# fhausmann/deepgrp

Measured on AMD Instinct MI355X. Metric: Mbp/sec predicted (whole node) at window=200 stride=50, 5-class, higher is better.
Workload: dtype f16

## Files before the change

deepgrp_amd/__main__.py:

```python
#!/usr/bin/env python3
from __future__ import annotations

import argparse
import logging
import os
import sys
from typing import Iterator, List, TextIO, Tuple

import numpy as np

logging.basicConfig()
_LOG = logging.getLogger(__name__)


def _read_multi_fasta(filestream: TextIO) -> Iterator[Tuple[str, str]]:
    from .fasta import read_multi_fasta_lines
    _LOG.debug("Reading FASTA file.")
    yield from read_multi_fasta_lines(filestream)


def _predict(dnasequence: str, model, options, step_size: int, use_mss: bool) -> Tuple[np.ndarray, int]:
    from .pipeline import ContigPipeline, upload_sequence
    _LOG.debug("One hot encoding sequence.")
    start_pos, d_idx = upload_sequence(dnasequence.encode("utf-8"))
# ... 379 lines not shown

    @staticmethod
    def _pipeline(args, options, model):
        from .pipeline import ContigPipeline
        pipe = ContigPipeline(model, args.step_size, options.batch_size, options.min_mss_len, options.xdrop_len,
                              use_mss=not args.no_use_mss, precise=getattr(args, "precise", False),
                              fast=getattr(args, "fast", False))
        _LOG.info("Forward kernel: %s", "plain fp32 kernels (more units than the fused kernels take)" if getattr(model, "fp32_only", False)
                  else "fused, split operands (fp32-grade)" if pipe.split else "fused, fp16 operands")
        return pipe

    _last_count = 0

    @staticmethod
    def _counted(records, _cb):
        from .fasta import DeviceRecord
        CommandLineParser._last_count = 0
        for header, rec in records:
            CommandLineParser._last_count += max(rec.length, 0) + max(rec.startpos, 0) if isinstance(rec, DeviceRecord) else len(rec)
            yield header, rec

    @staticmethod
    def _predict_tracked(pipe, runner, filename, records, outstream, kept, files, spec) -> int:
        from .evaluation import record_name
        from .runner import rows_text, rows_text_batch
        from .tracks import record_texts
        try:
            if _LOG.isEnabledFor(logging.DEBUG):
                bases = 0
                for chrom, (header, rec) in enumerate(records):
                    name = record_name(filename, header)
                    sink = lambda merged, startpos: files.write(record_texts(pipe, merged, startpos, name, spec, chrom))
                    rows, n = CommandLineParser._predict_staged(pipe, header, rec, sink)
                    if n == 0 and spec.bigwig:
# ... 406 lines not shown
```

deepgrp_amd/_lib.py:

```python
from __future__ import annotations

import ctypes as C
import os

_HERE = os.path.dirname(os.path.abspath(__file__))
LIB_PATH = os.path.join(_HERE, "libdeepgrp_hip.so")

i64, i32, vp, cint = C.c_int64, C.c_int32, C.c_void_p, C.c_int


class DgrpError(RuntimeError):
    """A libdeepgrp_hip call failed (message from dgrp_last_error())."""


class Segment(C.Structure):
    _fields_ = [("start", C.c_int64), ("end", C.c_int64), ("label", C.c_int32), ("contig", C.c_int32)]


_SIGNATURES = {
    "dgrp_abi_version": (cint, []),
    "dgrp_last_error": (C.c_char_p, []),
    "dgrp_device_info": (cint, [C.c_char_p, C.c_size_t, C.POINTER(cint), C.POINTER(i64)]),
    "dgrp_strip_n": (cint, [vp, i64, C.POINTER(i64), C.POINTER(i64)]),
    "dgrp_encode": (cint, [vp, i64, vp, vp]),
# ... 43 lines not shown
    "dgrp_forward_merge_record_workspace_bytes": (i64, [vp, i64, i64]),
    "dgrp_forward_reference_workspace_bytes": (i64, [vp, i64]),
    "dgrp_forward_windows_reference": (cint, [vp, vp, i64, i64, i64, i64, vp, vp, i64, vp]),
    "dgrp_get_max": (cint, [vp, i64, vp, i64, i64, i64, i64, vp]),
    "dgrp_scores": (cint, [vp, i64, cint, vp, vp, vp]),
    "dgrp_softmax_labels": (cint, [vp, i64, cint, vp, vp, vp, i64, vp]),
    "dgrp_mss_workspace_bytes": (i64, [i64]),
    "dgrp_mss_labels": (cint, [vp, vp, i64, cint, cint, cint, vp, vp, vp, i64, vp]),
    "dgrp_mss_segments_host": (cint, [vp, i64, vp, i64, C.POINTER(i64)]),
    "dgrp_mss_batch_workspace_bytes": (i64, [i64, i64]),
    "dgrp_mss_labels_batch": (cint, [vp, vp, i64, i64, vp, cint, cint, cint, vp, vp, i64, vp]),
    "dgrp_segments_workspace_bytes": (i64, [i64]),
    "dgrp_segments": (cint, [vp, i64, i64, i32, vp, i64, vp, vp, i64, vp]),
    "dgrp_record_workspace_bytes": (i64, [vp, i64, i64, cint]),
    "dgrp_predict_record": (cint, [vp, vp, i64, i64, i64, cint, cint, cint, i64, i32, vp, i64, C.POINTER(i64), vp, i64, vp]),
    "dgrp_batch_workspace_bytes": (i64, [vp, i64, vp, i64]),
    "dgrp_predict_batch": (cint, [vp, vp, i64, vp, vp, vp, vp, i64, i64, cint, cint, vp, i64, C.POINTER(i64), vp, i64, vp]),
    "dgrp_batch_rows": (i64, [i64, vp]),
    "dgrp_predict_batch_probs": (cint, [vp, vp, i64, vp, vp, vp, vp, i64, i64, cint, cint, vp, i64, C.POINTER(i64), vp, i64, vp, vp]),
    "dgrp_confusion_matrix": (cint, [vp, vp, i64, cint, vp, vp, vp]),
    "dgrp_filter_segments": (cint, [vp, vp, i64, i64, vp]),
    "dgrp_eval_workspace_bytes": (i64, [i64, i64]),
    "dgrp_paint_rows_batch": (cint, [vp, i64, vp, vp, vp, vp, vp, vp, i64, vp]),
    "dgrp_row_hits_batch": (cint, [vp, i64, vp, vp, vp, vp, vp, vp, vp, i64, vp]),
    "dgrp_row_scores_workspace_bytes": (i64, [i64, i64]),
    "dgrp_row_scores_batch": (cint, [vp, cint, i64, vp, vp, vp, vp, vp, vp, vp, i64, vp]),
    "dgrp_format_bed_bound": (i64, [i64, i64]),
    "dgrp_format_bed_rows": (cint, [vp, vp, i64, cint, vp, vp, i64, cint, vp, i64, C.POINTER(i64)]),
    "dgrp_inflate_raw_host": (cint, [vp, i64, vp, i64, C.POINTER(i64), C.POINTER(i64), C.POINTER(cint)]),
    "dgrp_inflate_workspace_bytes": (i64, [i64]),
# ... 43 lines not shown
```

deepgrp_amd/csrc/api.hip:

```cpp
#include "dgrp_model.h"

#include <stdarg.h>
#include <string.h>

#include <algorithm>
#include <vector>
#include <mutex>

static thread_local char g_err[512] = "";

void dgrp_set_error(const char *fmt, ...)
{
    va_list ap;
    va_start(ap, fmt);
    vsnprintf(g_err, sizeof(g_err), fmt, ap);
    va_end(ap);
}

DGRP_EXPORT int dgrp_abi_version(void) { return DGRP_ABI_VERSION; }
DGRP_EXPORT const char *dgrp_last_error(void) { return g_err; }

DGRP_EXPORT int dgrp_device_info(char *name, size_t name_cap, int *cu_count, int64_t *hbm_bytes)
{
    int dev = 0;
// ... 802 lines not shown
    l.count = take(8);
    l.fwd_bytes = record_forward_bytes(m, nwin);
    l.fwd = take(l.fwd_bytes);
    l.post_bytes = std::max<int64_t>(std::max<int64_t>(use_mss ? dgrp_mss_workspace_bytes(n) : 4096, dgrp_segments_workspace_bytes(n)), 4096);
    l.post = take(l.post_bytes);
    l.bytes = p;
    return l;
}

DGRP_EXPORT int64_t dgrp_record_workspace_bytes(const dgrp_model *m, int64_t n, int64_t s, int use_mss)
{
    if (!m || n < 0 || s < 1) return 0;
    return record_carve(m, n, s, use_mss).bytes;
}

DGRP_EXPORT int dgrp_predict_record(const dgrp_model *m, const uint8_t *d_idx, int64_t n, int64_t s, int64_t batch,
                                    int min_mss_len, int xdrop_len, int use_mss, int64_t offset, int32_t contig,
                                    dgrp_segment *d_records, int64_t cap, int64_t *h_count, void *d_work,
                                    int64_t work_bytes, void *stream_)
{
    hipStream_t stream = (hipStream_t)stream_;
    DGRP_REQUIRE(m && n >= 0 && s >= 1 && batch >= 1 && cap >= 0 && h_count, "dgrp_predict_record: bad arguments");
    *h_count = 0;
    if (n == 0) return DGRP_OK;
    DGRP_REQUIRE(d_idx && d_work && (cap == 0 || d_records), "dgrp_predict_record: NULL pointer");
    const record_layout l = record_carve(m, n, s, use_mss);
    if (work_bytes < l.bytes) {
        dgrp_set_error("dgrp_predict_record: workspace %lld < %lld bytes", (long long)work_bytes, (long long)l.bytes);
        return DGRP_ENOMEM;
    }
    char *w = (char *)d_work;
    float *out = (float *)(w + l.out);
    int8_t *labels = (int8_t *)(w + l.labels);
    int64_t *d_count = (int64_t *)(w + l.count);
    DGRP_HIP(hipMemsetAsync(out, 0, (size_t)n * m->C * 4, stream));
    int rc = dgrp_forward_merge_record(m, d_idx, n, s, batch, out, w + l.fwd, l.fwd_bytes, stream);
    if (rc) return rc;
    if (use_mss) {
        rc = dgrp_scores(out, n, m->C, (double *)(w + l.scores), (int8_t *)(w + l.cls), stream);
        if (rc) return rc;
        rc = dgrp_mss_labels((const double *)(w + l.scores), (const int8_t *)(w + l.cls), n, m->C, min_mss_len, xdrop_len,
                             labels, nullptr, w + l.post, l.post_bytes, stream);
    } else {
        rc = dgrp_softmax_labels(out, n, m->C, nullptr, labels, w + l.post, l.post_bytes, stream);
    }
    if (rc) return rc;
    rc = dgrp_segments(labels, n, offset, contig, d_records, cap, d_count, w + l.post, l.post_bytes, stream);
    if (rc) return rc;
    DGRP_HIP(hipMemcpyAsync(h_count, d_count, 8, hipMemcpyDeviceToHost, stream));
    DGRP_HIP(hipStreamSynchronize(stream));
    return DGRP_OK;
}

int dgrp_batch_marks(const int64_t *d_start, const int64_t *d_len, int64_t nrec, int64_t total_n, uint8_t *d_marks,
                     double *d_scores, int8_t *d_cls, hipStream_t stream);
int dgrp_batch_segments(const int8_t *d_labels, const uint8_t *d_marks, int64_t total_n, const int64_t *d_start, int64_t nrec,
                        const int64_t *d_startpos, const int32_t *d_contig, dgrp_segment *d_records, int64_t cap,
                        int64_t *d_count, void *d_work, int64_t work_bytes, hipStream_t stream);

struct batch_layout {
    int64_t out, scores, cls, labels, marks, count, recs, wgf, start, len, spos, contig, post, post_bytes, avg, pl, bytes;
};

static batch_layout batch_carve(const dgrp_model *m, int64_t nrec, int64_t total_rows, int64_t total_windows)
{
    batch_layout l;
// ... 142 lines not shown
```

deepgrp_amd/csrc/fasta_kernels.hip:

```cpp
#include "dgrp_common.h"
#include "scan.h"
#include <vector>
#include <algorithm>
#include <string.h>

__device__ __forceinline__ uint32_t fasta_class_of(uint32_t c)
{
    uint32_t l = c | 0x20u;
    return l == 'a' ? 0u : l == 'c' ? 1u : l == 'g' ? 2u : l == 't' ? 3u : 4u;
}

__global__ void __launch_bounds__(256) fasta_count_kernel(const uint8_t *__restrict__ raw, int64_t n, uint64_t *__restrict__ tilecnt,
                                                          unsigned long long *__restrict__ g)
{
    __shared__ uint64_t lds[4];
    const int64_t base = (int64_t)blockIdx.x * SCAN_TILE;
    uint64_t c = 0;
    bool bad = false;
    for (int j = 0; j < 8; ++j) {
        const int64_t i = base + j * 256 + threadIdx.x;
        if (i < n) {
            const uint32_t b = raw[i];
            const bool lineend = b == '\n' || b == '\r';
            c += lineend ? 0 : 1;
// ... 233 lines not shown
    if (word > 0) DGRP_HIP(hipMemcpyAsync(htiles.data(), tiles_base, (size_t)word * 8, hipMemcpyDeviceToHost, stream));
    DGRP_HIP(hipStreamSynchronize(stream));
    for (int64_t r = 0; r < nrec; ++r) {
        int64_t *info = h_info + 4 * r;
        if (h_len[r] == 0) { info[0] = 1; info[1] = 0; info[2] = 0; info[3] = 0; continue; }
        const unsigned long long *g = hg.data() + (size_t)r * 32;
        const int64_t tot = small[(size_t)r] ? (int64_t)g[3] : (int64_t)htiles[(size_t)grand_at[(size_t)r]];
        info[0] = g[0] ? 0 : 1;
        info[1] = tot;
        if (g[2] == 0) { info[2] = tot; info[3] = -tot; }
        else { info[2] = (int64_t)g[1]; info[3] = (int64_t)g[2] - (int64_t)g[1]; }
    }
    return DGRP_OK;
}

__global__ void __launch_bounds__(256) fasta_gt_kernel(const uint8_t *__restrict__ raw, int64_t n, int64_t cap,
                                                       unsigned long long *__restrict__ count, int64_t *__restrict__ list)
{
    const int64_t nvec = n / 16;
    for (int64_t v = (int64_t)blockIdx.x * blockDim.x + threadIdx.x; v <= nvec; v += (int64_t)gridDim.x * blockDim.x) {
        const int64_t p0 = v * 16;
        union { uint4 q; uint8_t b[16]; } u;
        uint8_t *b = u.b;
        int m = 16;
        if (v < nvec) {
            u.q = *(const uint4 *)(raw + p0);
        } else {
            m = (int)(n - p0);
            for (int j = 0; j < m; ++j) b[j] = raw[p0 + j];
        }
// ... 185 lines not shown
```

deepgrp_amd/fasta.py:

```python
from __future__ import annotations

import io
import mmap
import threading
import os
from typing import Iterator, List, Optional, TextIO, Tuple, Union

_DELETE = b"\n\r"
_ODD_WHITESPACE = (b" ", b"\t", b"\x0b", b"\x0c", b"\x1c", b"\x1d", b"\x1e", b"\x1f", b"\x85")


class LineLoop:

    __slots__ = ("header", "sequence", "opened", "key", "last_key")

    def __init__(self):
        self.header = ""
        self.sequence: List[str] = []
        self.opened = 0
        self.key = self.last_key = None

    def feed(self, lines, tag=None) -> Iterator[Tuple[str, str]]:
        for line in lines:
            line = line.strip()
# ... 100 lines not shown
    UPLOAD_STATS["bytes"] += int(size)
    UPLOAD_STATS["uploads"] += 1
    if size <= _SLAB:
        import numpy as np
        return torch.from_numpy(np.fromfile(path, dtype=np.uint8, count=size, offset=offset)).to(dev)
    key = (dev.index if dev.index is not None else torch.cuda.current_device())
    if key not in _UPLOAD:
        from concurrent.futures import ThreadPoolExecutor
        _UPLOAD[key] = ([torch.empty(_SLAB, dtype=torch.uint8, pin_memory=True) for _ in range(_NSLAB)], torch.cuda.Stream(device=dev),
                        ThreadPoolExecutor(max_workers=_NSLAB, thread_name_prefix="dgrp-upload"))
    slabs, copy, pool = _UPLOAD[key]
    with _UPLOAD_LOCK:
        return _upload_through(path, size, dev, slabs, copy, pool, offset)


def _upload_through(path, size: int, dev, slabs, copy, pool, offset: int = 0):
    import torch
    nslab = len(slabs)
    views = [b.numpy() for b in slabs]
    d_file = torch.empty(size, dtype=torch.uint8, device=dev)
    copy.wait_stream(torch.cuda.current_stream())
    fd = os.open(path, os.O_RDONLY)

    def reader(j):
        sent = None
        with torch.cuda.stream(copy):
            for o in range(j * _SLAB, size, nslab * _SLAB):
                want = min(_SLAB, size - o)
                if sent is not None:
                    sent.synchronize()
                got = 0
                while got < want:
                    k = os.preadv(fd, [views[j][got:want]], offset + o + got)
                    if not k:
                        raise OSError(f"{path}: shorter than its size at open ({offset + o + got} of {offset + size} bytes)")
                    got += k
                d_file[o:o + want].copy_(slabs[j][:want], non_blocking=True)
                sent = torch.cuda.Event()
                sent.record(copy)
        if sent is not None:
            sent.synchronize()

    try:
        jobs = [pool.submit(reader, j) for j in range(nslab)]
        err = None
        for job in jobs:
            try:
                job.result()
            except BaseException as e:
                err = err or e
        if err is not None:
            raise err
    finally:
        os.close(fd)
    torch.cuda.current_stream().wait_stream(copy)
    return d_file


def _device_chunks(L, d_file, size: int):
    import ctypes as C

    import numpy as np
    import torch

    from ._lib import check
    from .pipeline import stream_ptr
    cap = 4096
    while True:
        wb = L.dgrp_fasta_chunks_workspace_bytes(cap)
        work = torch.empty(wb, dtype=torch.uint8, device=d_file.device)
        st, lf, n = np.empty(cap, np.int64), np.empty(cap, np.int64), C.c_int64()
# ... 180 lines not shown
            work = torch.empty(wb, dtype=torch.uint8, device=dev)
            check(L.dgrp_fasta_encode_batch(d_raw.data_ptr(), c1 - c0, off.ctypes.data, ln.ctypes.data, d_idx.data_ptr(),
                                            infos.ctypes.data, work.data_ptr(), wb, stream_ptr()), "dgrp_fasta_encode_batch")
            del work
        if not keep_raw:
            d_raw = None
        grp = ChunkGroup()
        grp.c0, grp.c1, grp.starts, grp.head_ends, grp.body0s, grp.cand = c0, c1, starts, head_ends, body0s, cand
        grp.info, grp.d_idx, grp.d_raw = infos.tolist(), d_idx, d_raw
        del d_idx, d_raw
        yield grp
        del grp
        c0 = c1


def _ingest_range(L, dev, path, mm, r0: int, r1: int, group_bytes: int, group_records: int, d_file=None):
    loop = LineLoop()
    for grp in _chunk_groups(L, dev, path, mm, r0, r1, group_bytes, group_records, d_file=d_file):
        starts, head_ends, g0 = grp.starts, grp.head_ends, grp.starts[grp.c0]
        for i, c in enumerate(range(grp.c0, grp.c1)):
            a, b = r0 + starts[c], r0 + starts[c + 1]
            if grp.plain(i):
                for header, seq in loop.flush():
                    yield loop.last_key, header, seq
                header = mm[a:r0 + head_ends[c]].decode("ascii").strip()[1:]
                if header:
                    st, kept = grp.info[i][2], grp.info[i][3]
                    lo = grp.body0s[i] - g0 + st
                    yield (a, 0), header, DeviceRecord(st, None, kept, grp.d_idx, lo)
                continue
            for header, seq in loop.feed(_text_lines(mm[a:b]), tag=a):
# ... 5 lines not shown
```

deepgrp_amd/pipeline.py:

```python
from __future__ import annotations

import ctypes as C
from typing import NamedTuple, Optional, Tuple

import numpy as np
import torch

from ._lib import check, lib
from .fasta import DeviceRecord

SEGMENT_DTYPE = np.dtype([("start", "<i8"), ("end", "<i8"), ("label", "<i4"), ("contig", "<i4")])
ROW_SCORE_DTYPE = np.dtype([("sum", "<u8"), ("bases", "<i8"), ("agree", "<i8"), ("qmin", "<u4"), ("pad", "<u4")])


def require_gpu() -> torch.device:
    if not torch.cuda.is_available():
        raise RuntimeError("deepgrp_amd needs an AMD MI355X (gfx950) visible to PyTorch-ROCm; "
                           "there is no CPU fallback")
    return torch.device("cuda", torch.cuda.current_device())


def stream_ptr() -> int:
    return torch.cuda.current_stream().cuda_stream

# ... 373 lines not shown
        wb = L.dgrp_record_workspace_bytes(self.handle, n, self.step, int(self.use_mss))
        work = torch.empty(wb, dtype=torch.uint8, device=dev)
        cap = max(1024, n // 64)
        count = C.c_int64(0)
        while True:
            rec = torch.empty(cap * SEGMENT_DTYPE.itemsize, dtype=torch.uint8, device=dev)
            check(L.dgrp_predict_record(self.handle, _ptr(d_idx), n, self.step, self.batch, self.min_mss_len,
                                        self.xdrop_len, int(self.use_mss), int(startpos), int(contig), _ptr(rec), cap,
                                        C.byref(count), _ptr(work), wb, stream_ptr()), "dgrp_predict_record")
            if count.value <= cap:
                break
            cap = int(count.value)
        host = rec[: count.value * SEGMENT_DTYPE.itemsize].cpu().numpy()
        return host.view(SEGMENT_DTYPE).copy()

    def batchable(self) -> bool:
        return self.use_mss and self.event_log is None and not self.fp32 and not getattr(self.model, "fp32_only", False)

    def run_batch(self, d_base: torch.Tensor, offsets, lengths, startposes, contigs, d_probs: Optional[torch.Tensor] = None) -> np.ndarray:
        L = lib()
        nrec = len(lengths)
        if nrec == 0:
            return np.zeros(0, SEGMENT_DTYPE)
        off = np.ascontiguousarray(offsets, np.int64)
        ln = np.ascontiguousarray(lengths, np.int64)
        sp = np.ascontiguousarray(startposes, np.int64)
        cg = np.ascontiguousarray(contigs, np.int32)
        dev = d_base.device
        wb = L.dgrp_batch_workspace_bytes(self.handle, nrec, ln.ctypes.data, self.step)
        if wb <= 0:
# ... 259 lines not shown
```

deepgrp_amd/runner.py:

```python
from __future__ import annotations

import collections
import os
import threading
from concurrent.futures import ThreadPoolExecutor
from typing import Iterable, Iterator, List, NamedTuple, Tuple

import numpy as np
import torch

from .fasta import DeviceRecord
from .pipeline import ContigPipeline, record_indices

class _Tracked(NamedTuple):
    name: str
    rec: object
    chrom: int = 0


class _TrackedBatch(list):
    chrom0 = 0


class _Scored(NamedTuple):
    name: str
    rec: object
# ... 51 lines not shown
        return ""
    return _format(["{}\t{}\t".format(filename, h).encode("utf-8", "surrogateescape") for h in headers], True, rows)


class RecordRunner:

    def __init__(self, pipe: ContigPipeline, workers: int = 0, max_bases: int = 1 << 29, tracks=None):
        self.pipe = pipe
        self.tracks = tracks
        self.workers = workers or int(os.environ.get("DGRP_CLI_WORKERS", "16"))
        self.max_bases = max_bases
        m = pipe.model
        self._T, self._UP = m.vecsize, (m.units + 31) // 32 * 32

    def run_record(self, rec, contig: int = 0) -> np.ndarray:
        if isinstance(rec, DeviceRecord):
            startpos, d_idx = record_indices(rec)
            return self.pipe.run_idx(d_idx, startpos, contig)
        return self.pipe.run(rec, contig)

    def run_tracked(self, rec, name: str, chrom: int = 0):
        from .pipeline import SEGMENT_DTYPE
        from .tracks import empty_texts, record_texts
        startpos, d_idx = record_indices(rec)
        if d_idx.numel() == 0:
            return np.zeros(0, SEGMENT_DTYPE), empty_texts(self.tracks, name, startpos)
        merged = self.pipe.merged(d_idx)
        texts = record_texts(self.pipe, merged, startpos, name, self.tracks, chrom)
        return self.pipe.segments(self.pipe.labels(merged), startpos), texts

# ... 11 lines not shown

    def _batch_cost(self, n: int) -> int:
        cost = 80 * n
        m = self.pipe.model
        if self.tracks is not None:
            cost += 4 * m.classes * (n + 64) + len(self.tracks.classes) * (n // self.tracks.bin + 2) * (4 + 12 + 32)
        if m.attention:
            cost += len(range(0, n - self._T, self.pipe.step)) * self._T * (self._UP * 4 + m.classes * 4)
        return cost

    def work_items(self, records: Iterable[Tuple[object, object]]) -> Iterator[Tuple[object, object]]:
        group: List[Tuple[object, DeviceRecord]] = []
        cost = 0
        batchable = self.pipe.batchable()
        for key, rec in records:
            small = batchable and isinstance(rec, DeviceRecord) and rec.base is not None and 1 <= rec.length <= SMALL_RECORD
            if small:
                c = self._batch_cost(rec.length)
                if group and (group[0][1].base is not rec.base or len(group) >= BATCH_RECORDS or cost + c > BATCH_BYTES):
                    yield _BATCH, group
                    group, cost = [], 0
                group.append((key, rec))
                cost += c
            else:
                if group:
                    yield _BATCH, group
                    group, cost = [], 0
                yield key, rec
        if group:
            yield _BATCH, group
# ... 19 lines not shown
                texts = self.pipe.batch_track_texts(d_probs, row0, np.ascontiguousarray(lengths, np.int64), startposes,
                                                    [k[1] for k, _r in item], self.tracks, item.chrom0 if self.tracks.bigwig else 0)
            return [k for k, _r in item], rows, scores, texts
        if isinstance(item, list):
            rows = self.pipe.run_batch(item[0][1].base, [r.offset for _k, r in item], [r.length for _k, r in item],
                                       [r.startpos for _k, r in item], list(range(len(item))))
            return [k for k, _r in item], rows
        return self.run_record(item)

    @staticmethod
    def _size(item) -> int:
        if isinstance(item, (_Tracked, _Scored)):
            item = item.rec
        if isinstance(item, list):
            return sum(r.length for _k, r in item)
        return item.d_idx.numel() if isinstance(item, DeviceRecord) else len(item)

    def in_order(self, items: Iterable[Tuple[object, object]]) -> Iterator[Tuple[object, object]]:
        dev = torch.cuda.current_device() if torch.cuda.is_available() else None
        local = threading.local()
        taken = iter(range(self.workers))

        def task(item):
            if dev is None:
                return self.run_item(item)
            if not hasattr(local, "stream"):
                torch.cuda.set_device(dev)
                local.stream = _worker_stream(dev, next(taken))
            with torch.cuda.stream(local.stream):
                out = self.run_item(item)
# ... 67 lines not shown
```

include/deepgrp_hip.h:

```cpp
#ifndef DEEPGRP_HIP_H_
#define DEEPGRP_HIP_H_

#include <stddef.h>
#include <stdint.h>

#ifdef __cplusplus
extern "C" {
#endif

#define DGRP_OK 0
#define DGRP_EINVAL (-1)
#define DGRP_EHIP (-2)
#define DGRP_ENOMEM (-3)
#define DGRP_ENODEV (-4)

#define DGRP_ABI_VERSION 1

typedef struct dgrp_segment {
    int64_t start;
    int64_t end;
    int32_t label;
    int32_t contig;
} dgrp_segment;

// ... 147 lines not shown
                          dgrp_track_totals *h_totals, void *d_work, int64_t work_bytes, void *stream);

int64_t dgrp_zlib_bound(int64_t nblk, int64_t in_bytes);
int64_t dgrp_zlib_workspace_bytes(int64_t nblk, int level);
int dgrp_zlib_compress_batch(const uint8_t *d_in, int64_t in_bytes, const void *d_rows, int64_t stride, int64_t nblk, int level,
                             uint8_t *d_out, int64_t out_cap, int64_t *d_sizes, int64_t *h_out_bytes, void *d_work, int64_t work_bytes,
                             void *stream);
int dgrp_zlib_compress_host(const uint8_t *h_in, int64_t in_bytes, const void *h_rows, int64_t stride, int64_t nblk, int level,
                            uint8_t *h_out, int64_t out_cap, int64_t *h_sizes, int64_t *h_out_bytes);

int64_t dgrp_record_workspace_bytes(const dgrp_model *m, int64_t n, int64_t s, int use_mss);
int dgrp_predict_record(const dgrp_model *m, const uint8_t *d_idx, int64_t n, int64_t s, int64_t batch,
                        int min_mss_len, int xdrop_len, int use_mss, int64_t offset, int32_t contig,
                        dgrp_segment *d_records, int64_t cap, int64_t *h_count, void *d_work, int64_t work_bytes,
                        void *stream);

int64_t dgrp_batch_workspace_bytes(const dgrp_model *m, int64_t nrec, const int64_t *h_n, int64_t s);
int dgrp_predict_batch(const dgrp_model *m, const uint8_t *d_idx, int64_t nrec, const int64_t *h_idx_off,
                       const int64_t *h_n, const int64_t *h_startpos, const int32_t *h_contig, int64_t s, int64_t batch,
                       int min_mss_len, int xdrop_len, dgrp_segment *d_records, int64_t cap, int64_t *h_count,
                       void *d_work, int64_t work_bytes, void *stream);

int64_t dgrp_batch_rows(int64_t nrec, const int64_t *h_n);
int dgrp_predict_batch_probs(const dgrp_model *m, const uint8_t *d_idx, int64_t nrec, const int64_t *h_idx_off,
                             const int64_t *h_n, const int64_t *h_startpos, const int32_t *h_contig, int64_t s, int64_t batch,
                             int min_mss_len, int xdrop_len, dgrp_segment *d_records, int64_t cap, int64_t *h_count,
                             void *d_work, int64_t work_bytes, void *stream, float *d_probs);

int dgrp_confusion_matrix(const int8_t *d_true, const int8_t *d_pred, int64_t n, int ncls, int64_t *d_cnf,
                          int *d_bad, void *stream);
// ... 61 lines not shown
```

Baseline: 560.2.

## Stream large FASTA records in slabs and overlap encoding and GRU with upload

Large single-record FASTA files are now uploaded in slabs, and each slab is encoded on the device as soon as it arrives. GRU forward launches start on the windows already available while the rest of the file is still uploading, with a fallback that recomputes everything if the leading-N guess was wrong. This is meant to hide file upload and encoding time behind model compute for big chromosomes. It adds a new host/device handshake (ready flags, events, spin waits) and more complex record accounting, and it risks redundant work when the start-position guess misses.

```diff
diff --git a/deepgrp_amd/__main__.py b/deepgrp_amd/__main__.py
--- a/deepgrp_amd/__main__.py
+++ b/deepgrp_amd/__main__.py
@@ -417,10 +417,16 @@
 
     @staticmethod
     def _counted(records, _cb):
-        from .fasta import DeviceRecord
+        from .fasta import DeviceRecord, StreamedRecord
         CommandLineParser._last_count = 0
+
+        def add(n):
+            CommandLineParser._last_count += n
         for header, rec in records:
-            CommandLineParser._last_count += max(rec.length, 0) + max(rec.startpos, 0) if isinstance(rec, DeviceRecord) else len(rec)
+            if isinstance(rec, StreamedRecord) and rec.info is None:
+                rec.on_settle = lambda r: add(max(r.info[3], 0) + max(r.info[2], 0))
+            else:
+                add(max(rec.length, 0) + max(rec.startpos, 0) if isinstance(rec, DeviceRecord) else len(rec))
             yield header, rec
 
     @staticmethod
diff --git a/deepgrp_amd/_lib.py b/deepgrp_amd/_lib.py
--- a/deepgrp_amd/_lib.py
+++ b/deepgrp_amd/_lib.py
@@ -81,6 +81,11 @@
     "dgrp_segments": (cint, [vp, i64, i64, i32, vp, i64, vp, vp, i64, vp]),
     "dgrp_record_workspace_bytes": (i64, [vp, i64, i64, cint]),
     "dgrp_predict_record": (cint, [vp, vp, i64, i64, i64, cint, cint, cint, i64, i32, vp, i64, C.POINTER(i64), vp, i64, vp]),
+    "dgrp_stream_record_min_bytes": (i64, []),
+    "dgrp_stream_record_workspace_bytes": (i64, [vp, i64, i64, cint]),
+    "dgrp_predict_record_streamed": (cint, [vp, vp, i64, i64, vp, vp, vp, i64, i64, vp, i64, i64, cint, cint, cint, i32, vp, i64,
+                                            C.POINTER(i64), vp, vp, i64, vp]),
+    "dgrp_fasta_encode_slabs": (cint, [vp, i64, i64, vp, vp, vp, vp, i64, vp]),
     "dgrp_batch_workspace_bytes": (i64, [vp, i64, vp, i64]),
     "dgrp_predict_batch": (cint, [vp, vp, i64, vp, vp, vp, vp, i64, i64, cint, cint, vp, i64, C.POINTER(i64), vp, i64, vp]),
     "dgrp_batch_rows": (i64, [i64, vp]),
diff --git a/deepgrp_amd/csrc/api.hip b/deepgrp_amd/csrc/api.hip
--- a/deepgrp_amd/csrc/api.hip
+++ b/deepgrp_amd/csrc/api.hip
@@ -1,6 +1,7 @@
 #include "dgrp_model.h"
 
 #include <stdarg.h>
+#include <sched.h>
 #include <string.h>
 
 #include <algorithm>
@@ -840,6 +841,29 @@
     return record_carve(m, n, s, use_mss).bytes;
 }
 
+static int record_post(const dgrp_model *m, const record_layout &l, char *w, int64_t n, int min_mss_len, int xdrop_len, int use_mss,
+                       int64_t offset, int32_t contig, dgrp_segment *d_records, int64_t cap, int64_t *h_count, hipStream_t stream)
+{
+    float *out = (float *)(w + l.out);
+    int8_t *labels = (int8_t *)(w + l.labels);
+    int64_t *d_count = (int64_t *)(w + l.count);
+    int rc;
+    if (use_mss) {
+        rc = dgrp_scores(out, n, m->C, (double *)(w + l.scores), (int8_t *)(w + l.cls), stream);
+        if (rc) return rc;
+        rc = dgrp_mss_labels((const double *)(w + l.scores), (const int8_t *)(w + l.cls), n, m->C, min_mss_len, xdrop_len,
+                             labels, nullptr, w + l.post, l.post_bytes, stream);
+    } else {
+        rc = dgrp_softmax_labels(out, n, m->C, nullptr, labels, w + l.post, l.post_bytes, stream);
+    }
+    if (rc) return rc;
+    rc = dgrp_segments(labels, n, offset, contig, d_records, cap, d_count, w + l.post, l.post_bytes, stream);
+    if (rc) return rc;
+    DGRP_HIP(hipMemcpyAsync(h_count, d_count, 8, hipMemcpyDeviceToHost, stream));
+    DGRP_HIP(hipStreamSynchronize(stream));
+    return DGRP_OK;
+}
+
 DGRP_EXPORT int dgrp_predict_record(const dgrp_model *m, const uint8_t *d_idx, int64_t n, int64_t s, int64_t batch,
                                     int min_mss_len, int xdrop_len, int use_mss, int64_t offset, int32_t contig,
                                     dgrp_segment *d_records, int64_t cap, int64_t *h_count, void *d_work,
@@ -857,25 +881,140 @@
     }
     char *w = (char *)d_work;
     float *out = (float *)(w + l.out);
-    int8_t *labels = (int8_t *)(w + l.labels);
-    int64_t *d_count = (int64_t *)(w + l.count);
     DGRP_HIP(hipMemsetAsync(out, 0, (size_t)n * m->C * 4, stream));
     int rc = dgrp_forward_merge_record(m, d_idx, n, s, batch, out, w + l.fwd, l.fwd_bytes, stream);
     if (rc) return rc;
-    if (use_mss) {
-        rc = dgrp_scores(out, n, m->C, (double *)(w + l.scores), (int8_t *)(w + l.cls), stream);
+    return record_post(m, l, w, n, min_mss_len, xdrop_len, use_mss, offset, contig, d_records, cap, h_count, stream);
+}
+
+int dgrp_fasta_slab_begin(unsigned long long *d_st, int64_t n, hipStream_t stream);
+int dgrp_fasta_slab_ingest(const uint8_t *d_raw, int64_t a, int64_t b, int64_t n, uint8_t *d_idx, unsigned long long *d_st,
+                           uint64_t *d_tiles, hipStream_t stream);
+void dgrp_fasta_slab_info(const unsigned long long *h_st, int64_t *h_info);
+
+DGRP_EXPORT int64_t dgrp_stream_record_min_bytes(void)
+{
+    static const int64_t v = [] {
+        const char *e = getenv("DGRP_STREAM_MIN_BYTES");
+        if (!e || !e[0]) return (int64_t)(32ll << 20);
+        if (e[0] == 'o' || e[0] == 'O' || e[0] == '-') return (int64_t)-1;
+        return (int64_t)atoll(e);
+    }();
+    return v;
+}
+
+static int64_t round_windows()
+{
+    int dev = 0, cus = 0;
+    if (hipGetDevice(&dev) != hipSuccess || hipDeviceGetAttribute(&cus, hipDeviceAttributeMultiprocessorCount, dev) != hipSuccess || cus < 1)
+        cus = 256;
+    return 32ll * cus;
+}
+
+static int64_t stream_record_fasta_bytes(int64_t body_bytes)
+{
+    return dgrp_align_up(dgrp_fasta_workspace_bytes(body_bytes), 256);
+}
+
+DGRP_EXPORT int64_t dgrp_stream_record_workspace_bytes(const dgrp_model *m, int64_t body_bytes, int64_t s, int use_mss)
+{
+    if (!m || body_bytes < 0 || s < 1) return 0;
+    return record_carve(m, body_bytes, s, use_mss).bytes + stream_record_fasta_bytes(body_bytes);
+}
+
+DGRP_EXPORT int dgrp_predict_record_streamed(const dgrp_model *m, const uint8_t *d_body, int64_t body_bytes, int64_t nslab,
+                                             const int64_t *h_slab_end, void *const *h_events, const int32_t *h_ready,
+                                             int64_t startpos, int64_t range_windows, uint8_t *d_idx, int64_t s, int64_t batch,
+                                             int min_mss_len, int xdrop_len, int use_mss, int32_t contig, dgrp_segment *d_records,
+                                             int64_t cap, int64_t *h_count, int64_t *h_info, void *d_work, int64_t work_bytes,
+                                             void *stream_)
+{
+    hipStream_t stream = (hipStream_t)stream_;
+    DGRP_REQUIRE(m && body_bytes >= 0 && nslab >= 1 && h_slab_end && s >= 1 && batch >= 1 && cap >= 0 && h_count && h_info &&
+                 startpos >= 0 && range_windows >= 0, "dgrp_predict_record_streamed: bad arguments");
+    *h_count = 0;
+    h_info[0] = 1; h_info[1] = 0; h_info[2] = 0; h_info[3] = 0; h_info[4] = body_bytes;
+    int64_t prev = 0;
+    for (int64_t k = 0; k < nslab; ++k) {
+        DGRP_REQUIRE(h_slab_end[k] >= prev && h_slab_end[k] <= body_bytes, "dgrp_predict_record_streamed: slab ends must ascend within the body");
+        prev = h_slab_end[k];
+    }
+    DGRP_REQUIRE(prev == body_bytes, "dgrp_predict_record_streamed: the last slab must end at body_bytes");
+    if (body_bytes == 0) return DGRP_OK;
+    DGRP_REQUIRE(d_body && d_idx && d_work && (cap == 0 || d_records), "dgrp_predict_record_streamed: NULL pointer");
+    const record_layout l = record_carve(m, body_bytes, s, use_mss);
+    const int64_t need = l.bytes + stream_record_fasta_bytes(body_bytes);
+    if (work_bytes < need) {
+        dgrp_set_error("dgrp_predict_record_streamed: workspace %lld < %lld bytes", (long long)work_bytes, (long long)need);
+        return DGRP_ENOMEM;
+    }
+    char *w = (char *)d_work;
+    float *out = (float *)(w + l.out);
+    uint64_t *tiles = (uint64_t *)(w + l.bytes);
+    unsigned long long *st = (unsigned long long *)(w + need - 256);
+    const int64_t R = range_windows > 0 ? range_windows : round_windows();
+    const bool ranged = !m->ref_only && !m->attention;
+    const dgrp_placement early = { (int64_t)1 << 62, 0 };
+    DGRP_HIP(hipMemsetAsync(d_idx, 0, (size_t)body_bytes, stream));
+    DGRP_HIP(hipMemsetAsync(out, 0, (size_t)body_bytes * m->C * 4, stream));
+    int rc = dgrp_fasta_slab_begin(st, body_bytes, stream);
+    if (rc) return rc;
+    int64_t w_done = 0, ingested = 0;
+    prev = 0;
+    for (int64_t k = 0; k < nslab; ++k) {
+        if (h_ready) {
+            const volatile int32_t *flag = h_ready + k;
+            while (__atomic_load_n(flag, __ATOMIC_ACQUIRE) == 0) sched_yield();
+            if (*flag < 0) {
+                (void)hipStreamSynchronize(stream);
+                dgrp_set_error("dgrp_predict_record_streamed: the upload of slab %lld failed", (long long)k);
+                return DGRP_EINVAL;
+            }
+        }
+        if (h_events && h_events[k]) DGRP_HIP(hipStreamWaitEvent(stream, (hipEvent_t)h_events[k], 0));
+        prev = h_slab_end[k];
+        const bool last = k + 1 == nslab;
+        const int64_t avail_k = prev / 3 - startpos;
+        const int64_t wc_k = avail_k > 0 ? dgrp_window_count(avail_k, m->T, s) : 0;
+        const int64_t w1_k = wc_k / batch * batch / R * R;
+        if (!last && !(ranged && w1_k > w_done && (w_done == 0 || w1_k >= 4 * w_done))) continue;
+        rc = dgrp_fasta_slab_ingest(d_body, ingested, prev, body_bytes, d_idx, st, tiles, stream);
         if (rc) return rc;
-        rc = dgrp_mss_labels((const double *)(w + l.scores), (const int8_t *)(w + l.cls), n, m->C, min_mss_len, xdrop_len,
-                             labels, nullptr, w + l.post, l.post_bytes, stream);
+        ingested = prev;
+        if (!ranged || last) continue;
+        const int64_t avail = prev / 3 - startpos;
+        const int64_t wc = avail > 0 ? dgrp_window_count(avail, m->T, s) : 0;
+        const int64_t w1 = wc / batch * batch / R * R;
+        if (w1 > w_done && (w_done == 0 || w1 >= 4 * w_done)) {
+            rc = dgrp_gru_launch(m, dgrp_gru_plan_for(m, 0, s), d_idx + startpos, avail, early, w_done, w1 - w_done, out, nullptr, stream);
+            if (rc) return rc;
+            w_done = w1;
+        }
+    }
+    unsigned long long hst[8];
+    DGRP_HIP(hipMemcpyAsync(hst, st, sizeof(hst), hipMemcpyDeviceToHost, stream));
+    DGRP_HIP(hipStreamSynchronize(stream));
+    dgrp_fasta_slab_info(hst, h_info);
+    if (!h_info[0] || h_info[3] <= 0) return DGRP_OK;
+    const int64_t n = h_info[3];
+    const uint8_t *idx = d_idx + h_info[2];
+    const int64_t nwin = dgrp_window_count(n, m->T, s);
+    const dgrp_placement place = dgrp_make_placement(nwin, batch);
+    if (w_done > 0 && (h_info[2] != startpos || w_done > place.nfullB)) {
+        DGRP_HIP(hipMemsetAsync(out, 0, (size_t)n * m->C * 4, stream));
+        w_done = 0;
+    }
+    if (w_done == 0) {
+        rc = dgrp_forward_merge_record(m, idx, n, s, batch, out, w + l.fwd, l.fwd_bytes, stream);
+        if (rc) return rc;
     } else {
-        rc = dgrp_softmax_labels(out, n, m->C, nullptr, labels, w + l.post, l.post_bytes, stream);
-    }
-    if (rc) return rc;
-    rc = dgrp_segments(labels, n, offset, contig, d_records, cap, d_count, w + l.post, l.post_bytes, stream);
-    if (rc) return rc;
-    DGRP_HIP(hipMemcpyAsync(h_count, d_count, 8, hipMemcpyDeviceToHost, stream));
-    DGRP_HIP(hipStreamSynchronize(stream));
-    return DGRP_OK;
+        const int64_t chunk = record_window_chunk(m);
+        for (int64_t w0 = w_done; w0 < nwin; w0 += chunk) {
+            rc = dgrp_gru_launch(m, dgrp_gru_plan_for(m, 0, s), idx, n, place, w0, std::min<int64_t>(chunk, nwin - w0), out, nullptr, stream);
+            if (rc) return rc;
+        }
+    }
+    return record_post(m, l, w, n, min_mss_len, xdrop_len, use_mss, h_info[2], contig, d_records, cap, h_count, stream);
 }
 
 int dgrp_batch_marks(const int64_t *d_start, const int64_t *d_len, int64_t nrec, int64_t total_n, uint8_t *d_marks,
diff --git a/deepgrp_amd/csrc/fasta_kernels.hip b/deepgrp_amd/csrc/fasta_kernels.hip
--- a/deepgrp_amd/csrc/fasta_kernels.hip
+++ b/deepgrp_amd/csrc/fasta_kernels.hip
@@ -271,6 +271,157 @@
     return DGRP_OK;
 }
 
+__global__ void __launch_bounds__(256) fasta_slab_end_kernel(const uint8_t *__restrict__ raw, int64_t a, int64_t b,
+                                                             unsigned long long *__restrict__ st)
+{
+    for (int64_t i = a + (int64_t)blockIdx.x * blockDim.x + threadIdx.x; i < b; i += (int64_t)gridDim.x * blockDim.x)
+        if (raw[i] == '>' && (i == 0 || raw[i - 1] == '\n')) atomicMin(&st[4], (unsigned long long)i);
+}
+
+__global__ void __launch_bounds__(256) fasta_slab_count_kernel(const uint8_t *__restrict__ raw, int64_t a, int64_t b, int64_t n,
+                                                               uint64_t *__restrict__ tilecnt, unsigned long long *__restrict__ st)
+{
+    __shared__ uint64_t lds[4];
+    const int64_t end = (int64_t)st[4] < b ? (int64_t)st[4] : b;
+    const int64_t base = a + (int64_t)blockIdx.x * SCAN_TILE;
+    uint64_t c = 0;
+    bool bad = false;
+    for (int j = 0; j < 8; ++j) {
+        const int64_t i = base + j * 256 + threadIdx.x;
+        if (i < end) {
+            const uint32_t x = raw[i], p1 = i >= 1 ? raw[i - 1] : 0u, p2 = i >= 2 ? raw[i - 2] : 0u;
+            const bool lineend = x == '\n' || x == '\r';
+            c += lineend ? 0 : 1;
+            if (x >= 128 || (x <= 32 && !lineend)) bad = true;
+            if (lineend && i == 0) bad = true;
+            if (i >= 1 && p1 == '\r' && x != '\n') bad = true;
+            if (x == '\r' && i + 1 >= n) bad = true;
+            if (x == '\n' && i >= 1 && p1 == '\n') bad = true;
+            if (x == '\n' && i >= 2 && p1 == '\r' && p2 == '\n') bad = true;
+        }
+    }
+    for (int o = 32; o > 0; o >>= 1) c += __shfl_xor(c, o);
+    if ((threadIdx.x & 63) == 0) lds[threadIdx.x >> 6] = c;
+    if (__any(bad) && (threadIdx.x & 63) == 0) atomicOr(&st[0], 1ull);
+    __syncthreads();
+    if (threadIdx.x == 0) tilecnt[blockIdx.x] = lds[0] + lds[1] + lds[2] + lds[3];
+}
+
+__global__ void __launch_bounds__(256) fasta_slab_scatter_kernel(const uint8_t *__restrict__ raw, int64_t a, int64_t b,
+                                                                 const uint64_t *__restrict__ tileoff, uint8_t *__restrict__ idx,
+                                                                 unsigned long long *__restrict__ st)
+{
+    __shared__ uint64_t lds[4];
+    const int64_t end = (int64_t)st[4] < b ? (int64_t)st[4] : b;
+    const int64_t base = a + (int64_t)blockIdx.x * SCAN_TILE + (int64_t)threadIdx.x * 8;
+    uint32_t x[8];
+    uint64_t s = 0;
+    for (int j = 0; j < 8; ++j) {
+        x[j] = base + j < end ? raw[base + j] : (uint32_t)'\n';
+        s += (x[j] == '\n' || x[j] == '\r') ? 0 : 1;
+    }
+    uint64_t ex = block_exclusive_scan(s, nullptr, lds) + tileoff[blockIdx.x] + st[3];
+    long long first = 0x7fffffffffffffffll, last = -1;
+    for (int j = 0; j < 8; ++j) {
+        if (x[j] == '\n' || x[j] == '\r') continue;
+        idx[ex] = (uint8_t)fasta_class_of(x[j]);
+        if ((x[j] | 0x20u) != 'n') {
+            if ((long long)ex < first) first = (long long)ex;
+            last = (long long)ex + 1;
+        }
+        ++ex;
+    }
+    for (int o = 32; o > 0; o >>= 1) {
+        const long long f2 = __shfl_xor(first, o), l2 = __shfl_xor(last, o);
+        first = f2 < first ? f2 : first;
+        last = l2 > last ? l2 : last;
+    }
+    __shared__ long long red[8];
+    if ((threadIdx.x & 63) == 0) { red[threadIdx.x >> 6] = first; red[4 + (threadIdx.x >> 6)] = last; }
+    __syncthreads();
+    if (threadIdx.x == 0) {
+        for (int w = 1; w < 4; ++w) {
+            first = red[w] < first ? red[w] : first;
+            last = red[4 + w] > last ? red[4 + w] : last;
+        }
+        if (last >= 0) {
+            const volatile unsigned long long *gv = st;
+            if ((unsigned long long)first < gv[1]) atomicMin(&st[1], (unsigned long long)first);
+            if ((unsigned long long)last > gv[2]) atomicMax(&st[2], (unsigned long long)last);
+        }
+    }
+}
+
+__global__ void fasta_slab_advance_kernel(unsigned long long *__restrict__ st, const uint64_t *__restrict__ grand)
+{
+    if (threadIdx.x == 0 && blockIdx.x == 0) st[3] += *grand;
+}
+
+int dgrp_fasta_slab_begin(unsigned long long *d_st, int64_t n, hipStream_t stream)
+{
+    const unsigned long long init[8] = { 0ull, 0x7fffffffffffffffull, 0ull, 0ull, (unsigned long long)n, 0ull, 0ull, 0ull };
+    DGRP_HIP(hipMemcpyAsync(d_st, init, sizeof(init), hipMemcpyHostToDevice, stream));
+    return DGRP_OK;
+}
+
+int dgrp_fasta_slab_ingest(const uint8_t *d_raw, int64_t a, int64_t b, int64_t n, uint8_t *d_idx, unsigned long long *d_st,
+                           uint64_t *d_tiles, hipStream_t stream)
+{
+    if (b <= a) return DGRP_OK;
+    const int64_t ntiles = (b - a + SCAN_TILE - 1) / SCAN_TILE;
+    uint64_t *grand = d_tiles + ntiles + 1;
+    hipLaunchKernelGGL(fasta_slab_end_kernel, dim3((unsigned)grid_for(b - a, 256)), dim3(256), 0, stream, d_raw, a, b, d_st);
+    hipLaunchKernelGGL(fasta_slab_count_kernel, dim3((unsigned)ntiles), dim3(256), 0, stream, d_raw, a, b, n, d_tiles, d_st);
+    hipLaunchKernelGGL(scan_sums_kernel, dim3(1), dim3(256), 0, stream, d_tiles, ntiles, grand);
+    hipLaunchKernelGGL(fasta_slab_scatter_kernel, dim3((unsigned)ntiles), dim3(256), 0, stream, d_raw, a, b, d_tiles, d_idx, d_st);
+    hipLaunchKernelGGL(fasta_slab_advance_kernel, dim3(1), dim3(64), 0, stream, d_st, grand);
+    DGRP_LAUNCH_CHECK();
+    return DGRP_OK;
+}
+
+void dgrp_fasta_slab_info(const unsigned long long *h_st, int64_t *h_info)
+{
+    const int64_t total = (int64_t)h_st[3];
+    h_info[0] = h_st[0] ? 0 : 1;
+    h_info[1] = total;
+    if (h_st[2] == 0) { h_info[2] = total; h_info[3] = -total; }
+    else { h_info[2] = (int64_t)h_st[1]; h_info[3] = (int64_t)h_st[2] - (int64_t)h_st[1]; }
+    h_info[4] = (int64_t)h_st[4];
+}
+
+DGRP_EXPORT int dgrp_fasta_encode_slabs(const uint8_t *d_raw, int64_t nbytes, int64_t nslab, const int64_t *h_slab_end, uint8_t *d_idx,
+                                        int64_t *h_info, void *d_work, int64_t work_bytes, void *stream_)
+{
+    hipStream_t stream = (hipStream_t)stream_;
+    DGRP_REQUIRE(nbytes >= 0 && nslab >= 0 && h_info && (nslab == 0 || h_slab_end), "dgrp_fasta_encode_slabs: bad arguments");
+    h_info[0] = 1; h_info[1] = 0; h_info[2] = 0; h_info[3] = 0; h_info[4] = nbytes;
+    if (nbytes == 0) return DGRP_OK;
+    DGRP_REQUIRE(d_raw && d_idx && d_work, "dgrp_fasta_encode_slabs: NULL pointer");
+    int64_t prev = 0;
+    for (int64_t k = 0; k < nslab; ++k) {
+        DGRP_REQUIRE(h_slab_end[k] >= prev && h_slab_end[k] <= nbytes, "dgrp_fasta_encode_slabs: slab ends must ascend within the body");
+        prev = h_slab_end[k];
+    }
+    DGRP_REQUIRE(prev == nbytes, "dgrp_fasta_encode_slabs: the last slab must end at nbytes");
+    if (work_bytes < dgrp_fasta_workspace_bytes(nbytes)) {
+        dgrp_set_error("dgrp_fasta_encode_slabs: workspace too small");
+        return DGRP_ENOMEM;
+    }
+    unsigned long long *st = (unsigned long long *)((char *)d_work + dgrp_fasta_workspace_bytes(nbytes) - 256);
+    int rc = dgrp_fasta_slab_begin(st, nbytes, stream);
+    prev = 0;
+    for (int64_t k = 0; k < nslab && rc == DGRP_OK; ++k) {
+        rc = dgrp_fasta_slab_ingest(d_raw, prev, h_slab_end[k], nbytes, d_idx, st, (uint64_t *)d_work, stream);
+        prev = h_slab_end[k];
+    }
+    if (rc) return rc;
+    unsigned long long hst[8];
+    DGRP_HIP(hipMemcpyAsync(hst, st, sizeof(hst), hipMemcpyDeviceToHost, stream));
+    DGRP_HIP(hipStreamSynchronize(stream));
+    dgrp_fasta_slab_info(hst, h_info);
+    return DGRP_OK;
+}
+
 __global__ void __launch_bounds__(256) fasta_gt_kernel(const uint8_t *__restrict__ raw, int64_t n, int64_t cap,
                                                        unsigned long long *__restrict__ count, int64_t *__restrict__ list)
 {
diff --git a/deepgrp_amd/fasta.py b/deepgrp_amd/fasta.py
--- a/deepgrp_amd/fasta.py
+++ b/deepgrp_amd/fasta.py
@@ -138,7 +138,61 @@
         return _upload_through(path, size, dev, slabs, copy, pool, offset)
 
 
-def _upload_through(path, size: int, dev, slabs, copy, pool, offset: int = 0):
+class _Upload:
+
+    def __init__(self, d_file, size, events, ready, jobs, fd, copy):
+        self.d_file, self.size, self.events, self.ready = d_file, size, events, ready
+        self._jobs, self._fd, self._copy = jobs, fd, copy
+
+    def finish(self):
+        import torch
+        if self._jobs is None:
+            return
+        jobs, self._jobs = self._jobs, None
+        err = None
+        try:
+            for job in jobs:
+                try:
+                    job.result()
+                except BaseException as e:
+                    err = err or e
+        finally:
+            os.close(self._fd)
+            _UPLOAD_LOCK.release()
+        if err is not None:
+            raise err
+        torch.cuda.current_stream().wait_stream(self._copy)
+
+
+_EVENTS: dict = {}
+
+
+def _upload_start(path, size: int, dev, offset: int = 0) -> "_Upload":
+    import numpy as np
+    import torch
+    UPLOAD_STATS["bytes"] += int(size)
+    UPLOAD_STATS["uploads"] += 1
+    key = (dev.index if dev.index is not None else torch.cuda.current_device())
+    if key not in _UPLOAD:
+        from concurrent.futures import ThreadPoolExecutor
+        _UPLOAD[key] = ([torch.empty(_SLAB, dtype=torch.uint8, pin_memory=True) for _ in range(_NSLAB)], torch.cuda.Stream(device=dev),
+                        ThreadPoolExecutor(max_workers=_NSLAB, thread_name_prefix="dgrp-upload"))
+    slabs, copy, pool = _UPLOAD[key]
+    _UPLOAD_LOCK.acquire()
+    try:
+        npieces = (size + _SLAB - 1) // _SLAB
+        events = _EVENTS.setdefault(key, [])
+        while len(events) < npieces:
+            e = torch.cuda.Event()
+            e.record(copy)
+            events.append(e)
+        return _upload_through(path, size, dev, slabs, copy, pool, offset, events[:npieces], np.zeros(npieces, np.int32))
+    except BaseException:
+        _UPLOAD_LOCK.release()
+        raise
+
+
+def _upload_through(path, size: int, dev, slabs, copy, pool, offset: int = 0, events=None, ready=None):
     import torch
     nslab = len(slabs)
     views = [b.numpy() for b in slabs]
@@ -148,23 +202,36 @@
 
     def reader(j):
         sent = None
-        with torch.cuda.stream(copy):
-            for o in range(j * _SLAB, size, nslab * _SLAB):
-                want = min(_SLAB, size - o)
-                if sent is not None:
-                    sent.synchronize()
-                got = 0
-                while got < want:
-                    k = os.preadv(fd, [views[j][got:want]], offset + o + got)
-                    if not k:
-                        raise OSError(f"{path}: shorter than its size at open ({offset + o + got} of {offset + size} bytes)")
-                    got += k
-                d_file[o:o + want].copy_(slabs[j][:want], non_blocking=True)
-                sent = torch.cuda.Event()
-                sent.record(copy)
+        try:
+            with torch.cuda.stream(copy):
+                for o in range(j * _SLAB, size, nslab * _SLAB):
+                    want = min(_SLAB, size - o)
+                    if sent is not None:
+                        sent.synchronize()
+                    got = 0
+                    while got < want:
+                        k = os.preadv(fd, [views[j][got:want]], offset + o + got)
+                        if not k:
+                            raise OSError(f"{path}: shorter than its size at open ({offset + o + got} of {offset + size} bytes)")
+                        got += k
+                    d_file[o:o + want].copy_(slabs[j][:want], non_blocking=True)
+                    sent = events[o // _SLAB] if events is not None else torch.cuda.Event()
+                    sent.record(copy)
+                    if ready is not None:
+                        ready[o // _SLAB] = 1
+        except BaseException:
+            if ready is not None:
+                ready[j::nslab][ready[j::nslab] == 0] = -1
+            raise
         if sent is not None:
             sent.synchronize()
 
+    if events is not None:
+        try:
+            return _Upload(d_file, size, events, ready, [pool.submit(reader, j) for j in range(nslab)], fd, copy)
+        except BaseException:
+            os.close(fd)
+            raise
     try:
         jobs = [pool.submit(reader, j) for j in range(nslab)]
         err = None
@@ -179,6 +246,81 @@
         os.close(fd)
     torch.cuda.current_stream().wait_stream(copy)
     return d_file
+
+
+STREAM_MIN_BYTES = None
+
+
+def stream_min_bytes() -> int:
+    if STREAM_MIN_BYTES is not None:
+        return int(STREAM_MIN_BYTES)
+    from ._lib import lib
+    return int(lib().dgrp_stream_record_min_bytes())
+
+
+class StreamedRecord(DeviceRecord):
+
+    def __init__(self, path, a, up, body0, guess):
+        self.base, self.offset, self._view = None, 0, None
+        self.path, self.a, self.up, self.body0, self.guess = path, a, up, body0, guess
+        self.body_bytes = up.size - body0
+        self.lock, self.done = threading.Lock(), threading.Event()
+        self.runner_owned = False
+        self.info = None
+        self.on_settle = None
+
+    def settle(self, info, d_idx):
+        self.info = [int(v) for v in info]
+        self._view = d_idx[self.info[2]:self.info[2] + max(self.info[3], 0)] if d_idx is not None else None
+        if self.on_settle is not None:
+            self.on_settle(self)
+        self.done.set()
+
+    def materialize(self):
+        with self.lock:
+            if self.info is not None:
+                return
+            try:
+                import ctypes as C
+
+                import numpy as np
+                import torch
+
+                from ._lib import check, lib
+                from .pipeline import stream_ptr
+                L = lib()
+                self.up.finish()
+                n = self.body_bytes
+                d_idx = torch.empty(n, dtype=torch.uint8, device=self.up.d_file.device)
+                wb = L.dgrp_fasta_workspace_bytes(n)
+                work = torch.empty(wb, dtype=torch.uint8, device=d_idx.device)
+                info, ends = np.zeros(5, np.int64), np.array([n], np.int64)
+                check(L.dgrp_fasta_encode_slabs(self.up.d_file.data_ptr() + self.body0, n, 1, ends.ctypes.data, d_idx.data_ptr(),
+                                                info.ctypes.data, work.data_ptr(), wb, stream_ptr()), "dgrp_fasta_encode_slabs")
+                self.settle(info, d_idx)
+            finally:
+                self.done.set()
+
+    def text(self) -> str:
+        with open(self.path, "rb") as fh:
+            fh.seek(self.a)
+            raw = fh.read(self.body0 + self.info[4])
+        return next(read_multi_fasta_lines(_text_lines(raw)))[1]
+
+    @property
+    def startpos(self):
+        self.materialize()
+        return self.info[2]
+
+    @property
+    def length(self):
+        self.materialize()
+        return self.info[3]
+
+    @property
+    def d_idx(self):
+        self.materialize()
+        return self._view
 
 
 def _device_chunks(L, d_file, size: int):
@@ -389,7 +531,52 @@
         c0 = c1
 
 
-def _ingest_range(L, dev, path, mm, r0: int, r1: int, group_bytes: int, group_records: int, d_file=None):
+_NOT_N = None
+
+
+def _streamed_head(path, mm, dev, r0: int, r1: int):
+    global _NOT_N
+    size = r1 - r0
+    thr = stream_min_bytes()
+    if thr < 0 or size < thr or size <= _SLAB or size > RESIDENT_BYTES or mm[r0] != 62:
+        return None
+    lf = mm.find(b"\n", r0, min(r1, r0 + 65536))
+    if lf == -1 or lf + 1 >= r1:
+        return None
+    head = mm[r0:lf]
+    header = head.decode("ascii").strip()[1:] if head.isascii() and b"\r" not in head[:-1] else ""
+    if not header:
+        return None
+    if _NOT_N is None:
+        import re
+        _NOT_N = re.compile(rb"[^Nn\r\n]")
+    hit = _NOT_N.search(mm, lf + 1, r1)
+    stop = hit.start() if hit else r1
+    guess = stop - (lf + 1) - sum(mm[lf + 1:stop].count(c) for c in (b"\n", b"\r")) if stop > lf + 1 else 0
+    return header, StreamedRecord(path, r0, _upload_start(path, size, dev, r0), lf + 1 - r0, guess)
+
+
+def _ingest_range(L, dev, path, mm, r0: int, r1: int, group_bytes: int, group_records: int, d_file=None, stream_ok: bool = True):
+    got = _streamed_head(path, mm, dev, r0, r1) if d_file is None and stream_ok else None
+    if got is not None:
+        header, rec = got
+        try:
+            yield (r0, 0), header, rec
+        except GeneratorExit:
+            if rec.runner_owned:
+                rec.done.wait()
+            rec.up.finish()
+            raise
+        if rec.runner_owned:
+            rec.done.wait()
+        if rec.info is None:
+            rec.materialize()
+        rec.up.finish()
+        end = r0 + rec.body0 + rec.info[4]
+        d_all = rec.up.d_file
+        if end < r1:
+            yield from _ingest_range(L, dev, path, mm, end, r1, group_bytes, group_records, d_file=d_all[end - r0:].clone(), stream_ok=False)
+        return
     loop = LineLoop()
     for grp in _chunk_groups(L, dev, path, mm, r0, r1, group_bytes, group_records, d_file=d_file):
         starts, head_ends, g0 = grp.starts, grp.head_ends, grp.starts[grp.c0]
diff --git a/deepgrp_amd/pipeline.py b/deepgrp_amd/pipeline.py
--- a/deepgrp_amd/pipeline.py
+++ b/deepgrp_amd/pipeline.py
@@ -411,6 +411,40 @@
         host = rec[: count.value * SEGMENT_DTYPE.itemsize].cpu().numpy()
         return host.view(SEGMENT_DTYPE).copy()
 
+    def run_streamed(self, rec, contig: int = 0, range_windows: int = 0):
+        from .fasta import _SLAB
+        if self.event_log is not None or self.fp32:
+            return None
+        with rec.lock:
+            if rec.info is not None:
+                return None
+            try:
+                L = lib()
+                up, n = rec.up, rec.body_bytes
+                dev = up.d_file.device
+                wb = L.dgrp_stream_record_workspace_bytes(self.handle, n, self.step, int(self.use_mss))
+                work = torch.empty(wb, dtype=torch.uint8, device=dev)
+                d_idx = torch.empty(n, dtype=torch.uint8, device=dev)
+                cap = max(1024, n // 64)
+                out = torch.empty(cap * SEGMENT_DTYPE.itemsize, dtype=torch.uint8, device=dev)
+                npieces = len(up.events)
+                ends = np.minimum((np.arange(npieces, dtype=np.int64) + 1) * _SLAB, up.size) - rec.body0
+                events = (C.c_void_p * npieces)(*[e.cuda_event for e in up.events])
+                info, count = np.zeros(5, np.int64), C.c_int64(0)
+                check(L.dgrp_predict_record_streamed(self.handle, up.d_file.data_ptr() + rec.body0, n, npieces, ends.ctypes.data, events,
+                                                     up.ready.ctypes.data, int(rec.guess), int(range_windows), _ptr(d_idx), self.step,
+                                                     self.batch, self.min_mss_len, self.xdrop_len, int(self.use_mss), int(contig), _ptr(out),
+                                                     cap, C.byref(count), info.ctypes.data, _ptr(work), wb, stream_ptr()),
+                      "dgrp_predict_record_streamed")
+                up.finish()
+                rec.settle(info, d_idx)
+            finally:
+                rec.done.set()
+        if not info[0] or info[3] <= 0 or count.value > cap:
+            return None
+        host = out[: count.value * SEGMENT_DTYPE.itemsize].cpu().numpy()
+        return host.view(SEGMENT_DTYPE).copy()
+
     def batchable(self) -> bool:
         return self.use_mss and self.event_log is None and not self.fp32 and not getattr(self.model, "fp32_only", False)
 
diff --git a/deepgrp_amd/runner.py b/deepgrp_amd/runner.py
--- a/deepgrp_amd/runner.py
+++ b/deepgrp_amd/runner.py
@@ -9,7 +9,7 @@
 import numpy as np
 import torch
 
-from .fasta import DeviceRecord
+from .fasta import DeviceRecord, StreamedRecord
 from .pipeline import ContigPipeline, record_indices
 
 class _Tracked(NamedTuple):
@@ -91,6 +91,12 @@
         self._T, self._UP = m.vecsize, (m.units + 31) // 32 * 32
 
     def run_record(self, rec, contig: int = 0) -> np.ndarray:
+        if isinstance(rec, StreamedRecord):
+            rows = self.pipe.run_streamed(rec, contig)
+            if rows is not None:
+                return rows
+            if not rec.info[0]:
+                return self.pipe.run(rec.text(), contig)
         if isinstance(rec, DeviceRecord):
             startpos, d_idx = record_indices(rec)
             return self.pipe.run_idx(d_idx, startpos, contig)
@@ -132,6 +138,8 @@
         cost = 0
         batchable = self.pipe.batchable()
         for key, rec in records:
+            if isinstance(rec, StreamedRecord):
+                rec.runner_owned = True
             small = batchable and isinstance(rec, DeviceRecord) and rec.base is not None and 1 <= rec.length <= SMALL_RECORD
             if small:
                 c = self._batch_cost(rec.length)
@@ -181,6 +189,8 @@
             item = item.rec
         if isinstance(item, list):
             return sum(r.length for _k, r in item)
+        if isinstance(item, StreamedRecord):
+            return item.body_bytes
         return item.d_idx.numel() if isinstance(item, DeviceRecord) else len(item)
 
     def in_order(self, items: Iterable[Tuple[object, object]]) -> Iterator[Tuple[object, object]]:
diff --git a/include/deepgrp_hip.h b/include/deepgrp_hip.h
--- a/include/deepgrp_hip.h
+++ b/include/deepgrp_hip.h
@@ -185,6 +185,16 @@
                         int min_mss_len, int xdrop_len, int use_mss, int64_t offset, int32_t contig,
                         dgrp_segment *d_records, int64_t cap, int64_t *h_count, void *d_work, int64_t work_bytes,
                         void *stream);
+
+int64_t dgrp_stream_record_min_bytes(void);
+int64_t dgrp_stream_record_workspace_bytes(const dgrp_model *m, int64_t body_bytes, int64_t s, int use_mss);
+int dgrp_predict_record_streamed(const dgrp_model *m, const uint8_t *d_body, int64_t body_bytes, int64_t nslab,
+                                 const int64_t *h_slab_end, void *const *h_events, const int32_t *h_ready, int64_t startpos,
+                                 int64_t range_windows, uint8_t *d_idx, int64_t s, int64_t batch, int min_mss_len, int xdrop_len,
+                                 int use_mss, int32_t contig, dgrp_segment *d_records, int64_t cap, int64_t *h_count,
+                                 int64_t *h_info, void *d_work, int64_t work_bytes, void *stream);
+int dgrp_fasta_encode_slabs(const uint8_t *d_raw, int64_t nbytes, int64_t nslab, const int64_t *h_slab_end, uint8_t *d_idx,
+                            int64_t *h_info, void *d_work, int64_t work_bytes, void *stream);
 
 int64_t dgrp_batch_workspace_bytes(const dgrp_model *m, int64_t nrec, const int64_t *h_n, int64_t s);
 int dgrp_predict_batch(const dgrp_model *m, const uint8_t *d_idx, int64_t nrec, const int64_t *h_idx_off,
```

New measurement: 559.7. Within noise of the previous version (-0.1%).
